# ANRGUSC/DEFER

Measured on NVIDIA H100. Metric: inferences_per_sec, higher is better.
Workload: dtype bf16x3->f32

## Files before the change

### defer_b200/csrc/conv_umma.cu

```cuda
#include <cuda.h>
#include <string.h>

#include <type_traits>

#include <vector>

#include "common.cuh"
#include "conv_umma.cuh"

namespace defer {

static int env_int(const char* name, int dflt) {
  const char* v = getenv(name);
  return v ? atoi(v) : dflt;
}

namespace {

constexpr int BM = 128;
constexpr int BK = 64;
constexpr int CONS_THREADS = 256;
constexpr int NUM_THREADS = CONS_THREADS + 128;
constexpr int SMEM_CAP = 227 * 1024 - 256;
constexpr int CTL_BYTES = 256;
// ... 214 lines not shown
struct EpiArgs {
  const float* scale;
  const float* shift;
  const __nv_bfloat16* res;
  __nv_bfloat16* y;
  size_t plane;
  int cout;
  bool relu;
  bool store_first;
  bool relu2;
  const float* scale2;
  const float* shift2;
  __nv_bfloat16* y2;
};

__device__ __forceinline__ EpiArgs epi_args(const MegaOp& op) {
  const KParams& p = op.p;
  EpiArgs e;
  e.scale = p.scale;
  e.shift = p.shift;
  e.res = reinterpret_cast<const __nv_bfloat16*>(p.res);
  e.y = reinterpret_cast<__nv_bfloat16*>(p.y);
  e.plane = p.plane_out;
  e.cout = p.cout;
  e.relu = (p.flags & DEFER_FLAG_RELU) != 0;
  e.store_first = op.store_first != 0;
  e.relu2 = op.relu2 != 0;
  e.scale2 = op.scale2;
  e.shift2 = op.shift2;
  e.y2 = reinterpret_cast<__nv_bfloat16*>(op.y2);
  return e;
}

__device__ __forceinline__ uint32_t stg_off(int r, int c) {
  return (uint32_t)(r * STG_COLS + (((c >> 2) ^ ((r & 7) << 1)) << 2) + (c & 3)) * 4u;
}
__device__ __forceinline__ void sts2(uint32_t addr, float a, float b) {
  asm volatile("st.shared.v2.f32 [%0], {%1, %2};" ::"r"(addr), "f"(a), "f"(b));
}
__device__ __forceinline__ float4 lds4(uint32_t addr) {
  float4 v;
  asm volatile("ld.shared.v4.f32 {%0, %1, %2, %3}, [%4];" : "=f"(v.x), "=f"(v.y), "=f"(v.z), "=f"(v.w) : "r"(addr));
  return v;
}
__device__ __forceinline__ void stg4(void* p, uint4 v) {
  asm volatile("st.global.v4.b32 [%0], {%1, %2, %3, %4};" ::"l"(p), "r"(v.x), "r"(v.y), "r"(v.z), "r"(v.w));
}

__device__ __forceinline__ float bf_lo(uint32_t w) { return __uint_as_float(w << 16); }
__device__ __forceinline__ float bf_hi(uint32_t w) { return __uint_as_float(w & 0xffff0000u); }

template <int NPLANES, int BN, bool AFF>
__device__ __forceinline__ void epi_tile(const KParams& p, const EpiArgs& e, uint32_t stg, const float (&acc)[BN / 2],
                                         uint32_t qmask, int c_base, int n0, int h0, int w0) {
  const int tid = threadIdx.x;
  const int lane = tid & 31;
  const int row0 = (tid >> 7) * 64 + ((tid >> 5) & 3) * 16 + (lane >> 2);
  const int col_l = 2 * (lane & 3);
  const int jg = tid & 7;
  const int rb = tid >> 3;
  const int ca = 2 * jg + ((jg >> 2) & 1), cb = ca ^ 1;
  const bool swap = (jg >> 2) & 1;
  size_t orow[4];
  uint32_t vmask = 0;
#pragma unroll
  for (int k = 0; k < 4; ++k) {
    bool v;
    size_t pix;
    row_to_pixel(p, rb + 32 * k, n0, h0, w0, v, pix);
    orow[k] = pix * (size_t)e.cout;
    vmask |= (uint32_t)v << k;
  }
#pragma unroll
  for (int P = 0; P < BN / STG_COLS; ++P) {
    const bool mine = (qmask >> (8 * P + jg)) & 1u;
    const int c = c_base + STG_COLS * P + 8 * jg;
    cons_bar_sync();
#pragma unroll
    for (int qq = 0; qq < 8; ++qq) {
      const int q = 8 * P + qq;
      if (!((qmask >> q) & 1u)) continue;
      sts2(stg + stg_off(row0, 8 * qq + col_l), acc[4 * q], acc[4 * q + 1]);
      sts2(stg + stg_off(row0 + 8, 8 * qq + col_l), acc[4 * q + 2], acc[4 * q + 3]);
    }
    uint4 rh[4], rl[4];
#pragma unroll
    for (int k = 0; k < 4; ++k) {
      rh[k] = rl[k] = make_uint4(0u, 0u, 0u, 0u);
      if (e.res && mine && ((vmask >> k) & 1u)) {
        rh[k] = __ldcg(reinterpret_cast<const uint4*>(e.res + orow[k] + c));
        if (NPLANES == 2) rl[k] = __ldcg(reinterpret_cast<const uint4*>(e.res + e.plane + orow[k] + c));
      }
    }
    float sc[8], sf[8];
#pragma unroll
    for (int i = 0; i < 8; ++i) { sc[i] = 1.f; sf[i] = 0.f; }
    if (mine) {
      if (e.scale) {
        const float4 a = __ldg(reinterpret_cast<const float4*>(e.scale + c));
        const float4 b = __ldg(reinterpret_cast<const float4*>(e.scale + c + 4));
        sc[0] = a.x; sc[1] = a.y; sc[2] = a.z; sc[3] = a.w; sc[4] = b.x; sc[5] = b.y; sc[6] = b.z; sc[7] = b.w;
      }
      if (e.shift) {
        const float4 a = __ldg(reinterpret_cast<const float4*>(e.shift + c));
        const float4 b = __ldg(reinterpret_cast<const float4*>(e.shift + c + 4));
        sf[0] = a.x; sf[1] = a.y; sf[2] = a.z; sf[3] = a.w; sf[4] = b.x; sf[5] = b.y; sf[6] = b.z; sf[7] = b.w;
      }
    }
    cons_bar_sync();
    if (!mine) continue;

#pragma unroll
    for (int k = 0; k < 4; ++k) {
      if (!((vmask >> k) & 1u)) continue;
      const int r = rb + 32 * k;
      const float4 xa = lds4(stg + stg_off(r, 4 * ca));
      const float4 xb = lds4(stg + stg_off(r, 4 * cb));
      const float4 x0 = swap ? xb : xa, x1 = swap ? xa : xb;
      float v[8] = {x0.x, x0.y, x0.z, x0.w, x1.x, x1.y, x1.z, x1.w};
      const uint32_t hw[4] = {rh[k].x, rh[k].y, rh[k].z, rh[k].w};
      const uint32_t lw[4] = {rl[k].x, rl[k].y, rl[k].z, rl[k].w};
#pragma unroll
      for (int i = 0; i < 8; ++i) {
        v[i] = fmaf(v[i], sc[i], sf[i]);
        if (e.res) {
          v[i] += (i & 1) ? bf_hi(hw[i >> 1]) : bf_lo(hw[i >> 1]);
          if (NPLANES == 2) v[i] += (i & 1) ? bf_hi(lw[i >> 1]) : bf_lo(lw[i >> 1]);
        }
        if (e.relu) v[i] = fmaxf(v[i], 0.f);
      }
      uint4 hi, lo = make_uint4(0u, 0u, 0u, 0u);
      if (NPLANES == 2) {
        split_bf16x2(v[0], v[1], hi.x, lo.x);
        split_bf16x2(v[2], v[3], hi.y, lo.y);
        split_bf16x2(v[4], v[5], hi.z, lo.z);
        split_bf16x2(v[6], v[7], hi.w, lo.w);
      } else {
        hi = make_uint4(pack_bf16x2(v[0], v[1]), pack_bf16x2(v[2], v[3]), pack_bf16x2(v[4], v[5]), pack_bf16x2(v[6], v[7]));
      }
      const size_t o = orow[k] + c;
      if (!AFF || e.store_first) {
        stg4(e.y + o, hi);
        if (NPLANES == 2) stg4(e.y + e.plane + o, lo);
      }
      if constexpr (AFF) {
        float s2[8], t2[8];
        {
          const float4 a = __ldg(reinterpret_cast<const float4*>(e.scale2 + c));
          const float4 b = __ldg(reinterpret_cast<const float4*>(e.scale2 + c + 4));
          const float4 d = __ldg(reinterpret_cast<const float4*>(e.shift2 + c));
          const float4 f = __ldg(reinterpret_cast<const float4*>(e.shift2 + c + 4));
          s2[0] = a.x; s2[1] = a.y; s2[2] = a.z; s2[3] = a.w; s2[4] = b.x; s2[5] = b.y; s2[6] = b.z; s2[7] = b.w;
          t2[0] = d.x; t2[1] = d.y; t2[2] = d.z; t2[3] = d.w; t2[4] = f.x; t2[5] = f.y; t2[6] = f.z; t2[7] = f.w;
        }
        const uint32_t sh[4] = {hi.x, hi.y, hi.z, hi.w};
        const uint32_t sl[4] = {lo.x, lo.y, lo.z, lo.w};
        float u[8];
#pragma unroll
        for (int i = 0; i < 8; ++i) {
          u[i] = (i & 1) ? bf_hi(sh[i >> 1]) : bf_lo(sh[i >> 1]);
          if (NPLANES == 2) u[i] = u[i] + ((i & 1) ? bf_hi(sl[i >> 1]) : bf_lo(sl[i >> 1]));
          u[i] = fmaf(u[i], s2[i], t2[i]);
          if (e.relu2) u[i] = fmaxf(u[i], 0.f);
        }
        uint4 h2, l2;
        if (NPLANES == 2) {
          split_bf16x2(u[0], u[1], h2.x, l2.x);
          split_bf16x2(u[2], u[3], h2.y, l2.y);
          split_bf16x2(u[4], u[5], h2.z, l2.z);
          split_bf16x2(u[6], u[7], h2.w, l2.w);
          stg4(e.y2 + o, h2);
          stg4(e.y2 + e.plane + o, l2);
        } else {
          h2 = make_uint4(pack_bf16x2(u[0], u[1]), pack_bf16x2(u[2], u[3]), pack_bf16x2(u[4], u[5]), pack_bf16x2(u[6], u[7]));
          stg4(e.y2 + o, h2);
        }
      }
    }
  }
}

template <int NPLANES, int BN, int MODE, bool AFF = false>
__device__ __forceinline__ void conv_body(const MegaOp* ops, int n_ops, int stages, int pdl) {
  using L = Smem<NPLANES, BN>;
  constexpr int R = BN / 2;
  extern __shared__ uint8_t smem_raw[];
  uint8_t* smem = reinterpret_cast<uint8_t*>((reinterpret_cast<uintptr_t>(smem_raw) + 1023) & ~(uintptr_t)1023);
  const uint32_t ring = smem_u32(smem);
  const bool red = MODE == 0 && ops[0].p.cluster;
  const uint32_t stg = ring + L::ring(stages, red);
  const uint32_t bar_base = stg + STG_BYTES;
  auto full_bar = [&](int s) { return bar_base + 8u * s; };
  auto empty_bar = [&](int s) { return bar_base + 8u * (stages + s); };
  __shared__ int s_is_last;

  const int tid = threadIdx.x;
  if (tid == 0) {
    for (int s = 0; s < stages; ++s) {
      mbar_init(full_bar(s), 1);
      mbar_init(empty_bar(s), CONS_THREADS / 32);
    }
    asm volatile("fence.mbarrier_init.release.cluster;" ::: "memory");
  }
  __syncthreads();
  if (pdl) {
    asm volatile("griddepcontrol.wait;" ::: "memory");
    asm volatile("griddepcontrol.launch_dependents;" ::: "memory");
  }

  uint32_t it = 0;
  for (int o = 0; o < n_ops; ++o) {
    const MegaOp& op = ops[o];
    const KParams& p = op.p;
    const int total = op.m_tiles * op.n_tiles;
    int t_first, t_step;
    if (MODE == 0) {
      t_first = blockIdx.y * op.m_tiles + blockIdx.x;
      t_step = total;
    } else if (MODE == 1) {
      t_first = blockIdx.x;
      t_step = gridDim.x;
    } else {
      t_first = (int)cluster_ctarank();
      t_step = (int)cluster_nctarank();
    }
    const int split = MODE == 0 ? (int)blockIdx.z : 0;
    const int kb_begin = (split * p.k_blocks) / p.splits;
    const int kb_end = ((split + 1) * p.k_blocks) / p.splits;

    for (int t = t_first; t < total; t += t_step) {
      const int m_tile = t % op.m_tiles;
      const int c_base = (t / op.m_tiles) * BN;
      int n0 = 0, h0 = 0, w0 = 0;
      if (p.flat) {
        w0 = m_tile * BM;
      } else {
        const int tw = m_tile % p.tiles_w;
        const int t2 = m_tile / p.tiles_w;
        n0 = (t2 / p.tiles_h) * p.tile_n;
        h0 = (t2 % p.tiles_h) * p.tile_h;
        w0 = tw * p.tile_w;
      }

      if (tid >= CONS_THREADS) {
        if (tid == CONS_THREADS) {
          const uint32_t a_rows = p.flat ? (uint32_t)BM : (uint32_t)(p.tile_n * p.tile_h * p.tile_w);
          uint32_t i2 = it;
          for (int kb = kb_begin; kb < kb_end; ++kb, ++i2) {
            const int stage = (int)(i2 % (uint32_t)stages);
            const uint32_t phase = (i2 / (uint32_t)stages) & 1u;
            mbar_wait(empty_bar(stage), phase ^ 1u, 1);
            const uint32_t a_dst = ring + stage * L::STAGE;
            const uint32_t b_dst = a_dst + NPLANES * L::A_PLANE;
            const int tap = kb / p.cblocks;
            const int cb = kb - tap * p.cblocks;
            const int khi = tap / p.kw;
            const int kwi = tap - khi * p.kw;
            int cw = w0, ch = 0, cn = 0;
            if (!p.flat) {
              cw = w0 * p.sw + kwi - p.pad_l;
              ch = h0 * p.sh + khi - p.pad_t;
              cn = n0;
            }
            mbar_arrive_expect_tx(full_bar(stage), NPLANES * (a_rows * 128u + (uint32_t)L::B_PLANE));
            tma_load_4d(a_dst, &op.tmx[0], full_bar(stage), cb * BK, cw, ch, cn);
            tma_load_3d(b_dst, &op.tmw[0], full_bar(stage), cb * BK, c_base, tap);
            if (NPLANES == 2) {
              tma_load_4d(a_dst + L::A_PLANE, &op.tmx[1], full_bar(stage), cb * BK, cw, ch, cn);
              tma_load_3d(b_dst + L::B_PLANE, &op.tmw[1], full_bar(stage), cb * BK, c_base, tap);
            }
          }
        }
        it += (uint32_t)(kb_end - kb_begin);
        continue;
      }

      const int wg = tid >> 7;
      const int lane = tid & 31;
      float acc[R];
#pragma unroll
      for (int i = 0; i < R; ++i) acc[i] = 0.f;
      int prev_stage = -1;
      for (int kb = kb_begin; kb < kb_end; ++kb, ++it) {
        const int stage = (int)(it % (uint32_t)stages);
        mbar_wait(full_bar(stage), (it / (uint32_t)stages) & 1u, 2);
        const uint32_t a_addr = ring + stage * L::STAGE + wg * (64 * 128);
        const uint32_t b_addr = ring + stage * L::STAGE + NPLANES * L::A_PLANE;
        wg_fence();
#pragma unroll
        for (int k = 0; k < BK / 16; ++k) {
          const uint64_t a_hi = make_sw128_desc(a_addr + k * 32);
          const uint64_t b_hi = make_sw128_desc(b_addr + k * 32);
          wgmma_bf16<BN>(acc, a_hi, b_hi);
          if (NPLANES == 2) {
            wgmma_bf16<BN>(acc, make_sw128_desc(a_addr + L::A_PLANE + k * 32), b_hi);
            wgmma_bf16<BN>(acc, a_hi, make_sw128_desc(b_addr + L::B_PLANE + k * 32));
          }
        }
        wg_commit();
        wg_wait<1>();
        acc_fence(acc);
        if (prev_stage >= 0 && lane == 0) mbar_arrive(empty_bar(prev_stage));
        prev_stage = stage;
      }
      wg_wait<0>();
      acc_fence(acc);
      if (prev_stage >= 0 && lane == 0) mbar_arrive(empty_bar(prev_stage));


      if (MODE == 0 && p.cluster) {
        cons_bar_sync();
        float4* red_buf = reinterpret_cast<float4*>(smem);
#pragma unroll
        for (int q = 0; q < R / 4; ++q)
          red_buf[q * CONS_THREADS + tid] = make_float4(acc[4 * q], acc[4 * q + 1], acc[4 * q + 2], acc[4 * q + 3]);
        break;
      }
      if (MODE == 0 && p.splits > 1) {
        const size_t tile_lin = (size_t)t;
        float4* mine = reinterpret_cast<float4*>(p.partial) + (tile_lin * p.splits + split) * (R / 4) * CONS_THREADS;
#pragma unroll
        for (int q = 0; q < R / 4; ++q)
          __stcg(mine + q * CONS_THREADS + tid, make_float4(acc[4 * q], acc[4 * q + 1], acc[4 * q + 2], acc[4 * q + 3]));
        __threadfence();
        cons_bar_sync();
        if (tid == 0) {
          const unsigned prev = atomicAdd(p.counters + tile_lin, 1u);
          const int last = prev == (unsigned)(p.splits - 1);
          if (last) p.counters[tile_lin] = 0;
          s_is_last = last;
        }
        cons_bar_sync();
        if (!s_is_last) continue;
        __threadfence();
#pragma unroll
        for (int i = 0; i < R; ++i) acc[i] = 0.f;
        for (int s = 0; s < p.splits; ++s) {
          const float4* src = reinterpret_cast<const float4*>(p.partial) + (tile_lin * p.splits + s) * (R / 4) * CONS_THREADS;
#pragma unroll
          for (int q = 0; q < R / 4; ++q) {
            const float4 v = __ldcg(src + q * CONS_THREADS + tid);
            acc[4 * q] += v.x; acc[4 * q + 1] += v.y; acc[4 * q + 2] += v.z; acc[4 * q + 3] += v.w;
          }
        }
      }
      epi_tile<NPLANES, BN, AFF>(p, epi_args(op), stg, acc, 0xffffu, c_base, n0, h0, w0);
    }

    if (MODE == 0 && p.cluster) {
      cluster_sync_all();
      if (tid < CONS_THREADS) {
        const int m_tile = blockIdx.x;
        int n0 = 0, h0 = 0, w0 = 0;
        if (p.flat) {
          w0 = m_tile * BM;
        } else {
          const int t2 = m_tile / p.tiles_w;
          n0 = (t2 / p.tiles_h) * p.tile_n;
          h0 = (t2 % p.tiles_h) * p.tile_h;
          w0 = (m_tile % p.tiles_w) * p.tile_w;
        }
        const int S = p.splits;
        const int rank = (int)cluster_ctarank();
        const uint32_t mine = ring + (uint32_t)tid * 16u;
        float acc[R];
        uint32_t qmask = 0;
#pragma unroll
        for (int q = 0; q < R / 4; ++q) {
          acc[4 * q] = acc[4 * q + 1] = acc[4 * q + 2] = acc[4 * q + 3] = 0.f;
          if (q % S != rank) continue;
          qmask |= 1u << q;
          const uint32_t addr = mine + (uint32_t)(q * CONS_THREADS) * 16u;
          float4 a = dsmem_ld4(dsmem_map(addr, 0));
          for (int s = 1; s < S; ++s) {
            const float4 v = dsmem_ld4(dsmem_map(addr, (uint32_t)s));
            a.x += v.x; a.y += v.y; a.z += v.z; a.w += v.w;
          }
          acc[4 * q] = a.x; acc[4 * q + 1] = a.y; acc[4 * q + 2] = a.z; acc[4 * q + 3] = a.w;
        }
        epi_tile<NPLANES, BN, AFF>(p, epi_args(op), stg, acc, qmask, (int)blockIdx.y * BN, n0, h0, w0);
      }
      cluster_sync_all();
    }
    if (MODE == 2 && o + 1 < n_ops) {
      asm volatile("fence.proxy.async.global;" ::: "memory");
      cluster_sync_all();
    }
  }
}

template <int NPLANES, int BN>
__global__ void __launch_bounds__(NUM_THREADS, 1) conv_umma_kernel(const __grid_constant__ MegaOp op, int stages, int pdl) {
  conv_body<NPLANES, BN, 0>(&op, 1, stages, pdl);
}

template <int NPLANES, int BN>
__global__ void __launch_bounds__(NUM_THREADS, 1) conv_stream_kernel(const MegaOp* __restrict__ ops, int stages, int pdl) {
  conv_body<NPLANES, BN, 1>(ops, 1, stages, pdl);
}

template <int NPLANES, int BN>
__global__ void __launch_bounds__(NUM_THREADS, 1) conv_umma_aff_kernel(const __grid_constant__ MegaOp op, int stages, int pdl) {
  conv_body<NPLANES, BN, 0, true>(&op, 1, stages, pdl);
}

template <int NPLANES, int BN>
__global__ void __launch_bounds__(NUM_THREADS, 1) conv_stream_aff_kernel(const MegaOp* __restrict__ ops, int stages, int pdl) {
  conv_body<NPLANES, BN, 1, true>(ops, 1, stages, pdl);
}

template <int NPLANES>
__global__ void __launch_bounds__(NUM_THREADS, 1) conv_mega_kernel(const MegaOp* __restrict__ ops, int n_ops, int stages) {
  conv_body<NPLANES, MEGA_BN, 2>(ops, n_ops, stages, 0);
}

enum StemIn { STEM_F32, STEM_U8_CAFFE, STEM_U8_TF };
constexpr int PROD_THREADS = NUM_THREADS - CONS_THREADS;
constexpr int STEM_WIN_BYTES = 24 * 1024;
constexpr int STEM_WIN_VALS = STEM_WIN_BYTES / 4;
constexpr int STEM_FILL = STEM_WIN_VALS / PROD_THREADS;
constexpr int STEM_TILE_W = 16;

template <int NPLANES>
struct StemSmem {
  static constexpr int STAGE = Smem<NPLANES, 64>::STAGE;
  __host__ __device__ static constexpr int total(int stages) {
    return stages * STAGE + STG_BYTES + 2 * STEM_WIN_BYTES + CTL_BYTES + 1024;
  }
  __host__ __device__ static constexpr int max_stages() {
    return (SMEM_CAP - STG_BYTES - 2 * STEM_WIN_BYTES - CTL_BYTES - 1024) / STAGE > MAX_STAGES
               ? MAX_STAGES
               : (SMEM_CAP - STG_BYTES - 2 * STEM_WIN_BYTES - CTL_BYTES - 1024) / STAGE;
  }
};
static_assert(StemSmem<2>::max_stages() == 3 && StemSmem<1>::max_stages() == 6, "stem ring depths with two image windows");
static_assert(STEM_FILL * PROD_THREADS == STEM_WIN_VALS, "the producer threads cover a whole window");

struct StemGeo {
  const float* x;
  const uint8_t* u8;
  float s0, s1, s2;
// ... 145 lines not shown
    int wb = 0;
    for (int t = blockIdx.x; t < total; t += gridDim.x, wb ^= 1) {
      const int t_next = t + (int)gridDim.x;
      if (t_next < total) {
        stem_tile_origin(p, t_next % op.m_tiles, n0, h0, w0);
        stem_fill_load<IN>(g, ptid, n0, h0, w0, raw);
      }
      prod_bar_sync();
      const uint32_t win = win0 + (uint32_t)wb * STEM_WIN_BYTES;
      const int c_base = (t / op.m_tiles) * 64;
      for (int kb = 0; kb < k_blocks; ++kb, ++it) {
        const int stage = (int)(it % (uint32_t)stages);
        mbar_wait(empty_bar(stage), ((it / (uint32_t)stages) & 1u) ^ 1u, 1);
        const uint32_t a_dst = ring + stage * L::STAGE;
        const uint32_t b_dst = a_dst + NPLANES * L::A_PLANE;
        if (ptid == 0) {
          mbar_expect_tx(full_bar(stage), NPLANES * (uint32_t)L::B_PLANE);
          tma_load_3d(b_dst, &op.tmw[0], full_bar(stage), kb * BK, c_base, 0);
          if (NPLANES == 2) tma_load_3d(b_dst + L::B_PLANE, &op.tmw[1], full_bar(stage), kb * BK, c_base, 0);
        }
        stem_build<NPLANES>(g, win, a_dst, ptid, row_base, kb);
        asm volatile("fence.proxy.async.shared::cta;" ::: "memory");
        prod_bar_sync();
        if (ptid == 0) mbar_arrive(full_bar(stage));
      }
      if (t_next < total) stem_fill_store<IN>(g, win0 + (uint32_t)(wb ^ 1) * STEM_WIN_BYTES, ptid, raw);
    }
    return;
  }

  const int wg = tid >> 7;
  const int lane = tid & 31;
  for (int t = blockIdx.x; t < total; t += gridDim.x) {
    float acc[32];
#pragma unroll
    for (int i = 0; i < 32; ++i) acc[i] = 0.f;
    int prev_stage = -1;
    for (int kb = 0; kb < k_blocks; ++kb, ++it) {
      const int stage = (int)(it % (uint32_t)stages);
      mbar_wait(full_bar(stage), (it / (uint32_t)stages) & 1u, 2);
      const uint32_t a_addr = ring + stage * L::STAGE + wg * (64 * 128);
      const uint32_t b_addr = ring + stage * L::STAGE + NPLANES * L::A_PLANE;
      wg_fence();
#pragma unroll
      for (int k = 0; k < BK / 16; ++k) {
        const uint64_t a_hi = make_sw128_desc(a_addr + k * 32);
        const uint64_t b_hi = make_sw128_desc(b_addr + k * 32);
        wgmma_bf16<64>(acc, a_hi, b_hi);
        if (NPLANES == 2) {
          wgmma_bf16<64>(acc, make_sw128_desc(a_addr + L::A_PLANE + k * 32), b_hi);
          wgmma_bf16<64>(acc, a_hi, make_sw128_desc(b_addr + L::B_PLANE + k * 32));
        }
      }
      wg_commit();
      wg_wait<1>();
      acc_fence(acc);
      if (prev_stage >= 0 && lane == 0) mbar_arrive(empty_bar(prev_stage));
      prev_stage = stage;
    }
    wg_wait<0>();
    acc_fence(acc);
    if (prev_stage >= 0 && lane == 0) mbar_arrive(empty_bar(prev_stage));
    int n0, h0, w0;
    stem_tile_origin(p, t % op.m_tiles, n0, h0, w0);
    epi_tile<NPLANES, 64, false>(p, epi_args(op), stg, acc, 0xffffu, (t / op.m_tiles) * 64, n0, h0, w0);
  }
}

template <int NPLANES>
__global__ void __launch_bounds__(NUM_THREADS, 1) conv_stem_kernel(const MegaOp* __restrict__ ops, int stages, int pdl) {
  stem_body<NPLANES, STEM_F32>(ops, stages, pdl);
}

template <int NPLANES>
__global__ void __launch_bounds__(NUM_THREADS, 1) conv_stem_u8_kernel(const MegaOp* __restrict__ ops, int stages, int pdl) {
  stem_body<NPLANES, STEM_U8_CAFFE>(ops, stages, pdl);
}

template <int NPLANES>
__global__ void __launch_bounds__(NUM_THREADS, 1) conv_stem_u8tf_kernel(const MegaOp* __restrict__ ops, int stages, int pdl) {
  stem_body<NPLANES, STEM_U8_TF>(ops, stages, pdl);
}

__global__ void __launch_bounds__(256) weight_transform_kernel(const float* __restrict__ w, __nv_bfloat16* __restrict__ out,
                                                               int taps, int cin, int cout, int nplanes) {
  size_t total = (size_t)taps * cin * cout;
  size_t i = (size_t)blockIdx.x * blockDim.x + threadIdx.x;
  if (i >= total) return;
  int ci = (int)(i % cin);
  size_t t2 = i / cin;
  int co = (int)(t2 % cout);
  int tap = (int)(t2 / cout);
  float v = w[((size_t)tap * cin + ci) * cout + co];
  __nv_bfloat16 hi = __float2bfloat16_rn(v);
// ... 132 lines not shown
  kernel<<<grid, NUM_THREADS, smem, st>>>(op, stages, 0);
  DEFER_CUDA(cudaGetLastError());
  return DEFER_OK;
}

template <auto kernel>
int launch_grid(const void* dev_op, int n_tiles, int stages, size_t smem, cudaStream_t st) {
  DEFER_TRY((set_smem_attr<kernel>()));
  const int sms = sm_count();
  int grid = sms < n_tiles ? sms : n_tiles;
  const int rounds = (n_tiles + grid - 1) / grid;
  grid = (n_tiles + rounds - 1) / rounds;
  static const int pdl = env_int("DEFER_PDL", 0);
  if (pdl) {
    cudaLaunchConfig_t cfg;
    memset(&cfg, 0, sizeof cfg);
    cfg.gridDim = dim3(grid, 1, 1);
    cfg.blockDim = dim3(NUM_THREADS, 1, 1);
    cfg.dynamicSmemBytes = smem;
    cfg.stream = st;
    cudaLaunchAttribute attr[1];
    attr[0].id = cudaLaunchAttributeProgrammaticStreamSerialization;
    attr[0].val.programmaticStreamSerializationAllowed = 1;
    cfg.attrs = attr;
    cfg.numAttrs = 1;
    DEFER_CUDA(cudaLaunchKernelEx(&cfg, kernel, reinterpret_cast<const MegaOp*>(dev_op), stages, 1));
    return DEFER_OK;
  }
  kernel<<<grid, NUM_THREADS, smem, st>>>(reinterpret_cast<const MegaOp*>(dev_op), stages, 0);
  DEFER_CUDA(cudaGetLastError());
  return DEFER_OK;
}

template <int NPLANES, int BN, bool AFF = false>
int launch_persist_t(const void* dev_op, int n_tiles, int stages, cudaStream_t st) {
  using L = Smem<NPLANES, BN>;
  constexpr auto kernel = AFF ? &conv_stream_aff_kernel<NPLANES, BN> : &conv_stream_kernel<NPLANES, BN>;
  if (stages > L::max_stages()) stages = L::max_stages();
  if (stages < 2) stages = 2;
  return launch_grid<kernel>(dev_op, n_tiles, stages, (size_t)L::total(stages, false), st);
}

template <int NPLANES, int IN>
int launch_stem_t(const void* dev_op, int n_tiles, int stages, cudaStream_t st) {
  using L = StemSmem<NPLANES>;
  constexpr auto kernel = IN == STEM_U8_TF      ? &conv_stem_u8tf_kernel<NPLANES>
                          : IN == STEM_U8_CAFFE ? &conv_stem_u8_kernel<NPLANES>
                                                : &conv_stem_kernel<NPLANES>;
  if (stages > L::max_stages()) stages = L::max_stages();
  if (stages < 2) stages = 2;
  return launch_grid<kernel>(dev_op, n_tiles, stages, (size_t)L::total(stages), st);
}

template <int NPLANES>
int launch_mega_t(const void* dev_ops, int n_ops, int stages, cudaStream_t st) {
  using L = Smem<NPLANES, MEGA_BN>;
  DEFER_TRY(set_smem_attr<conv_mega_kernel<NPLANES>>(true));
  if (stages < 2) stages = 2;
  if (stages > L::max_stages()) stages = L::max_stages();
  const int cluster = umma_mega_cluster_size();
  cudaLaunchConfig_t cfg;
  memset(&cfg, 0, sizeof cfg);
  cfg.gridDim = dim3(cluster, 1, 1);
  cfg.blockDim = dim3(NUM_THREADS, 1, 1);
  cfg.dynamicSmemBytes = L::total(stages, false);
  cfg.stream = st;
  cudaLaunchAttribute attr[1];
  attr[0].id = cudaLaunchAttributeClusterDimension;
  attr[0].val.clusterDim.x = cluster;
  attr[0].val.clusterDim.y = 1;
// ... 187 lines not shown
}

size_t umma_mega_op_bytes() { return sizeof(MegaOp); }

int umma_mega_fill(void* host_dst, const UmmaConvPlan& P, const UmmaConvLaneArgs& a) {
  if (!P.ready || (P.bn != MEGA_BN && !P.stream) || P.splits != 1) {
    set_error("umma_mega_fill: plan is not a persistent-kernel plan (bn %d, splits %d)", P.bn, P.splits);
    return DEFER_ERR_STATE;
  }
  MegaOp op;
  fill_op(P, a, &op);
  memcpy(host_dst, &op, sizeof op);
  return DEFER_OK;
}

int umma_mega_cluster_size() {
  static int cached = 0;
  if (cached) return cached;
  int want = env_int("DEFER_MEGA_CLUSTER", 8);
  if (want < 1) want = 1;
  if (want > 16) want = 16;
  cached = want;
  return cached;
}

int launch_conv_persistent(int nplanes, const void* dev_op, int n_tiles, bool aff, cudaStream_t st) {
  const int stages = env_int("DEFER_PERSIST_STAGES", MAX_STAGES);
  if (aff)
    return nplanes == 2 ? launch_persist_t<2, 64, true>(dev_op, n_tiles, stages, st)
                        : launch_persist_t<1, 64, true>(dev_op, n_tiles, stages, st);
  return nplanes == 2 ? launch_persist_t<2, 64>(dev_op, n_tiles, stages, st) : launch_persist_t<1, 64>(dev_op, n_tiles, stages, st);
}

int launch_conv_stream(int nplanes, int bn, const void* dev_op, int n_tiles, int k_blocks, bool aff, cudaStream_t st) {
  (void)k_blocks;
  const int stages = env_int("DEFER_STREAM_STAGES", MAX_STAGES);
  if (aff) {
    if (bn == 128) return nplanes == 2 ? launch_persist_t<2, 128, true>(dev_op, n_tiles, stages, st)
                                       : launch_persist_t<1, 128, true>(dev_op, n_tiles, stages, st);
    if (bn == 64) return nplanes == 2 ? launch_persist_t<2, 64, true>(dev_op, n_tiles, stages, st)
                                      : launch_persist_t<1, 64, true>(dev_op, n_tiles, stages, st);
  }
  if (bn == 128) return nplanes == 2 ? launch_persist_t<2, 128>(dev_op, n_tiles, stages, st) : launch_persist_t<1, 128>(dev_op, n_tiles, stages, st);
  if (bn == 64) return nplanes == 2 ? launch_persist_t<2, 64>(dev_op, n_tiles, stages, st) : launch_persist_t<1, 64>(dev_op, n_tiles, stages, st);
  set_error("conv_stream: unsupported N tile %d", bn);
  return DEFER_ERR_INVALID;
}

static void stem_tile(int ho, int wo, int kh, int kw, int sh, int sw, int cin, int* tile_h, int* tile_w, int* win_rows,
                      int* win_cols) {
  *tile_w = wo < STEM_TILE_W ? wo : STEM_TILE_W;
  *tile_h = BM / *tile_w < ho ? BM / *tile_w : ho;
  *win_rows = (*tile_h - 1) * sh + kh;
  *win_cols = ((*tile_w - 1) * sw + kw) * cin;
}

bool umma_stem_fusable(int fmt, int cin, int ho, int wo, int cout, int kh, int kw, int sh, int sw, uint32_t flags) {
  if (fmt != FMT_BF16X2 && fmt != FMT_BF16) return false;
  if (cout != 64 || (flags & DEFER_FLAG_RESIDUAL) || kh * kw * cin > 256) return false;
  int tile_h, tile_w, win_rows, win_cols;
  stem_tile(ho, wo, kh, kw, sh, sw, cin, &tile_h, &tile_w, &win_rows, &win_cols);
  return (long long)win_rows * win_cols <= STEM_WIN_VALS;
}

int umma_mega_set_stem(void* host_op, const float* x, int h, int w, int cin, int kh, int kw, int sh, int sw, int pad_t,
                       int pad_l) {
  MegaOp* op = reinterpret_cast<MegaOp*>(host_op);
  KParams& p = op->p;
  op->stem_x = x;
  op->stem_h = h; op->stem_w = w; op->stem_cin = cin;
  op->stem_kh = kh; op->stem_kw = kw; op->stem_sh = sh; op->stem_sw = sw;
  op->stem_pad_t = pad_t; op->stem_pad_l = pad_l;
  op->stem_K = kh * kw * cin;
  stem_tile(p.ho, p.wo, kh, kw, sh, sw, cin, &p.tile_h, &p.tile_w, &op->stem_win_rows, &op->stem_win_cols);
  p.flat = 0;
  p.tile_n = 1;
  p.tiles_h = (p.ho + p.tile_h - 1) / p.tile_h;
// ... 36 lines not shown
```

Baseline: 14220.

## Add ping-pong consumer warpgroup schedule and residual L2 prefetch to stream conv

Adds an optional ping-pong mode for the persistent stream conv kernel. Each consumer warpgroup computes a full 128-row tile on alternating tiles, ordered by mbarriers, so one group's epilogue overlaps the other's MMA. Register budgets are redistributed with setmaxnreg. It also adds an L2 prefetch of the residual tile before the mainloop, which runs in stream mode regardless of the ping-pong setting. Ping-pong is selected by an environment variable that defaults off, so its extra complexity and register pressure only apply when enabled.

```diff
diff --git a/defer_b200/csrc/conv_umma.cu b/defer_b200/csrc/conv_umma.cu
--- a/defer_b200/csrc/conv_umma.cu
+++ b/defer_b200/csrc/conv_umma.cu
@@ -270,8 +270,27 @@
   return e;
 }
 
+template <int NPLANES, int BN, int G>
+__device__ __forceinline__ void prefetch_res_tile(const KParams& p, int c_base, int n0, int h0, int w0) {
+  const __nv_bfloat16* res = reinterpret_cast<const __nv_bfloat16*>(p.res);
+  if (!res) return;
+  constexpr int LINES = BM * (BN / 64) * NPLANES;
+  const int gt = threadIdx.x % G;
+#pragma unroll
+  for (int i = 0; i < (LINES + G - 1) / G; ++i) {
+    const int l = gt + i * G;
+    if (l >= LINES) break;
+    const int r = l % BM, q = (l / BM) % (BN / 64), pl = l / (BM * (BN / 64));
+    bool v;
+    size_t pix;
+    row_to_pixel(p, r, n0, h0, w0, v, pix);
+    if (v) asm volatile("prefetch.global.L2 [%0];" ::"l"(res + pl * p.plane_out + pix * (size_t)p.cout + c_base + 64 * q));
+  }
+}
+
+template <int SC>
 __device__ __forceinline__ uint32_t stg_off(int r, int c) {
-  return (uint32_t)(r * STG_COLS + (((c >> 2) ^ ((r & 7) << 1)) << 2) + (c & 3)) * 4u;
+  return (uint32_t)(r * SC + (((c >> 2) ^ ((r & (SC / 8 - 1)) << 1)) << 2) + (c & 3)) * 4u;
 }
 __device__ __forceinline__ void sts2(uint32_t addr, float a, float b) {
   asm volatile("st.shared.v2.f32 [%0], {%1, %2};" ::"r"(addr), "f"(a), "f"(b));
@@ -288,17 +307,25 @@
 __device__ __forceinline__ float bf_lo(uint32_t w) { return __uint_as_float(w << 16); }
 __device__ __forceinline__ float bf_hi(uint32_t w) { return __uint_as_float(w & 0xffff0000u); }
 
-template <int NPLANES, int BN, bool AFF>
-__device__ __forceinline__ void epi_tile(const KParams& p, const EpiArgs& e, uint32_t stg, const float (&acc)[BN / 2],
-                                         uint32_t qmask, int c_base, int n0, int h0, int w0) {
+template <int NPLANES, int BN, bool AFF, int G = CONS_THREADS>
+__device__ __forceinline__ void epi_tile(const KParams& p, const EpiArgs& e, uint32_t stg,
+                                         const float (&acc)[CONS_THREADS / G][BN / 2], uint32_t qmask, int c_base, int n0,
+                                         int h0, int w0) {
+  static_assert(G == CONS_THREADS || G == 128, "an epilogue group is both consumer warpgroups or one");
+  constexpr int H = CONS_THREADS / G;
+  constexpr int SC = G / 4;
+  constexpr int JG = SC / 8;
   const int tid = threadIdx.x;
+  const int gt = tid % G;
   const int lane = tid & 31;
-  const int row0 = (tid >> 7) * 64 + ((tid >> 5) & 3) * 16 + (lane >> 2);
+  const int row0 = (gt >> 7) * 64 + ((gt >> 5) & 3) * 16 + (lane >> 2);
   const int col_l = 2 * (lane & 3);
-  const int jg = tid & 7;
-  const int rb = tid >> 3;
-  const int ca = 2 * jg + ((jg >> 2) & 1), cb = ca ^ 1;
-  const bool swap = (jg >> 2) & 1;
+  const int jg = gt % JG;
+  const int rb = gt / JG;
+  const bool swap = (gt >> 2) & 1;
+  const int ca = 2 * jg + swap, cb = ca ^ 1;
+  const uint32_t bar = G == CONS_THREADS ? 1u : 3u + (uint32_t)(tid >> 7);
+  if (G != CONS_THREADS) stg += (uint32_t)(tid >> 7) * (uint32_t)(BM * SC * 4);
   size_t orow[4];
   uint32_t vmask = 0;
 #pragma unroll
@@ -310,16 +337,19 @@
     vmask |= (uint32_t)v << k;
   }
 #pragma unroll
-  for (int P = 0; P < BN / STG_COLS; ++P) {
-    const bool mine = (qmask >> (8 * P + jg)) & 1u;
-    const int c = c_base + STG_COLS * P + 8 * jg;
-    cons_bar_sync();
-#pragma unroll
-    for (int qq = 0; qq < 8; ++qq) {
-      const int q = 8 * P + qq;
+  for (int P = 0; P < BN / SC; ++P) {
+    const bool mine = (qmask >> (JG * P + jg)) & 1u;
+    const int c = c_base + SC * P + 8 * jg;
+    asm volatile("bar.sync %0, %1;" ::"r"(bar), "n"(G) : "memory");
+#pragma unroll
+    for (int qq = 0; qq < JG; ++qq) {
+      const int q = JG * P + qq;
       if (!((qmask >> q) & 1u)) continue;
-      sts2(stg + stg_off(row0, 8 * qq + col_l), acc[4 * q], acc[4 * q + 1]);
-      sts2(stg + stg_off(row0 + 8, 8 * qq + col_l), acc[4 * q + 2], acc[4 * q + 3]);
+#pragma unroll
+      for (int h = 0; h < H; ++h) {
+        sts2(stg + stg_off<SC>(row0 + 64 * h, 8 * qq + col_l), acc[h][4 * q], acc[h][4 * q + 1]);
+        sts2(stg + stg_off<SC>(row0 + 64 * h + 8, 8 * qq + col_l), acc[h][4 * q + 2], acc[h][4 * q + 3]);
+      }
     }
     uint4 rh[4], rl[4];
 #pragma unroll
@@ -345,15 +375,15 @@
         sf[0] = a.x; sf[1] = a.y; sf[2] = a.z; sf[3] = a.w; sf[4] = b.x; sf[5] = b.y; sf[6] = b.z; sf[7] = b.w;
       }
     }
-    cons_bar_sync();
+    asm volatile("bar.sync %0, %1;" ::"r"(bar), "n"(G) : "memory");
     if (!mine) continue;
 
 #pragma unroll
     for (int k = 0; k < 4; ++k) {
       if (!((vmask >> k) & 1u)) continue;
       const int r = rb + 32 * k;
-      const float4 xa = lds4(stg + stg_off(r, 4 * ca));
-      const float4 xb = lds4(stg + stg_off(r, 4 * cb));
+      const float4 xa = lds4(stg + stg_off<SC>(r, 4 * ca));
+      const float4 xb = lds4(stg + stg_off<SC>(r, 4 * cb));
       const float4 x0 = swap ? xb : xa, x1 = swap ? xa : xb;
       float v[8] = {x0.x, x0.y, x0.z, x0.w, x1.x, x1.y, x1.z, x1.w};
       const uint32_t hw[4] = {rh[k].x, rh[k].y, rh[k].z, rh[k].w};
@@ -418,10 +448,15 @@
   }
 }
 
-template <int NPLANES, int BN, int MODE, bool AFF = false>
+enum { WALK_ALL, WALK_PRODUCER, WALK_CONSUMERS };
+
+template <int NPLANES, int BN, int MODE, bool AFF = false, bool PINGPONG = false>
 __device__ __forceinline__ void conv_body(const MegaOp* ops, int n_ops, int stages, int pdl) {
   using L = Smem<NPLANES, BN>;
   constexpr int R = BN / 2;
+  constexpr bool PP = MODE == 1 && PINGPONG;
+  constexpr int H = PP ? 2 : 1;
+  constexpr int EPI_G = PP ? 128 : CONS_THREADS;
   extern __shared__ uint8_t smem_raw[];
   uint8_t* smem = reinterpret_cast<uint8_t*>((reinterpret_cast<uintptr_t>(smem_raw) + 1023) & ~(uintptr_t)1023);
   const uint32_t ring = smem_u32(smem);
@@ -430,13 +465,18 @@
   const uint32_t bar_base = stg + STG_BYTES;
   auto full_bar = [&](int s) { return bar_base + 8u * s; };
   auto empty_bar = [&](int s) { return bar_base + 8u * (stages + s); };
+  auto ord_bar = [&](int g) { return bar_base + 8u * (2 * stages + g); };
   __shared__ int s_is_last;
 
   const int tid = threadIdx.x;
   if (tid == 0) {
     for (int s = 0; s < stages; ++s) {
       mbar_init(full_bar(s), 1);
-      mbar_init(empty_bar(s), CONS_THREADS / 32);
+      mbar_init(empty_bar(s), EPI_G / 32);
+    }
+    if (PP) {
+      mbar_init(ord_bar(0), 1);
+      mbar_init(ord_bar(1), 1);
     }
     asm volatile("fence.mbarrier_init.release.cluster;" ::: "memory");
   }
@@ -445,185 +485,215 @@
     asm volatile("griddepcontrol.wait;" ::: "memory");
     asm volatile("griddepcontrol.launch_dependents;" ::: "memory");
   }
-
-  uint32_t it = 0;
-  for (int o = 0; o < n_ops; ++o) {
-    const MegaOp& op = ops[o];
-    const KParams& p = op.p;
-    const int total = op.m_tiles * op.n_tiles;
-    int t_first, t_step;
-    if (MODE == 0) {
-      t_first = blockIdx.y * op.m_tiles + blockIdx.x;
-      t_step = total;
-    } else if (MODE == 1) {
-      t_first = blockIdx.x;
-      t_step = gridDim.x;
-    } else {
-      t_first = (int)cluster_ctarank();
-      t_step = (int)cluster_nctarank();
-    }
-    const int split = MODE == 0 ? (int)blockIdx.z : 0;
-    const int kb_begin = (split * p.k_blocks) / p.splits;
-    const int kb_end = ((split + 1) * p.k_blocks) / p.splits;
-
-    for (int t = t_first; t < total; t += t_step) {
-      const int m_tile = t % op.m_tiles;
-      const int c_base = (t / op.m_tiles) * BN;
-      int n0 = 0, h0 = 0, w0 = 0;
-      if (p.flat) {
-        w0 = m_tile * BM;
+  auto walk = [&](auto role) {
+    constexpr int ROLE = decltype(role)::value;
+    uint32_t it = 0;
+    for (int o = 0; o < n_ops; ++o) {
+      const MegaOp& op = ops[o];
+      const KParams& p = op.p;
+      const int total = op.m_tiles * op.n_tiles;
+      int t_first, t_step;
+      if (MODE == 0) {
+        t_first = blockIdx.y * op.m_tiles + blockIdx.x;
+        t_step = total;
+      } else if (MODE == 1) {
+        t_first = blockIdx.x;
+        t_step = gridDim.x;
       } else {
-        const int tw = m_tile % p.tiles_w;
-        const int t2 = m_tile / p.tiles_w;
-        n0 = (t2 / p.tiles_h) * p.tile_n;
-        h0 = (t2 % p.tiles_h) * p.tile_h;
-        w0 = tw * p.tile_w;
+        t_first = (int)cluster_ctarank();
+        t_step = (int)cluster_nctarank();
       }
-
-      if (tid >= CONS_THREADS) {
-        if (tid == CONS_THREADS) {
-          const uint32_t a_rows = p.flat ? (uint32_t)BM : (uint32_t)(p.tile_n * p.tile_h * p.tile_w);
-          uint32_t i2 = it;
-          for (int kb = kb_begin; kb < kb_end; ++kb, ++i2) {
-            const int stage = (int)(i2 % (uint32_t)stages);
-            const uint32_t phase = (i2 / (uint32_t)stages) & 1u;
-            mbar_wait(empty_bar(stage), phase ^ 1u, 1);
-            const uint32_t a_dst = ring + stage * L::STAGE;
-            const uint32_t b_dst = a_dst + NPLANES * L::A_PLANE;
-            const int tap = kb / p.cblocks;
-            const int cb = kb - tap * p.cblocks;
-            const int khi = tap / p.kw;
-            const int kwi = tap - khi * p.kw;
-            int cw = w0, ch = 0, cn = 0;
-            if (!p.flat) {
-              cw = w0 * p.sw + kwi - p.pad_l;
-              ch = h0 * p.sh + khi - p.pad_t;
-              cn = n0;
+      const int split = MODE == 0 ? (int)blockIdx.z : 0;
+      const int kb_begin = (split * p.k_blocks) / p.splits;
+      const int kb_end = ((split + 1) * p.k_blocks) / p.splits;
+
+      auto origin = [&](int t, int& c_base, int& n0, int& h0, int& w0) {
+        const int m_tile = PP ? t / op.n_tiles : t % op.m_tiles;
+        c_base = (PP ? t % op.n_tiles : t / op.m_tiles) * BN;
+        n0 = h0 = w0 = 0;
+        if (p.flat) {
+          w0 = m_tile * BM;
+        } else {
+          const int tw = m_tile % p.tiles_w;
+          const int t2 = m_tile / p.tiles_w;
+          n0 = (t2 / p.tiles_h) * p.tile_n;
+          h0 = (t2 % p.tiles_h) * p.tile_h;
+          w0 = tw * p.tile_w;
+        }
+      };
+
+      for (int t = t_first, j = 0; t < total; t += t_step, ++j) {
+        int c_base, n0, h0, w0;
+        origin(t, c_base, n0, h0, w0);
+
+        if (ROLE == WALK_PRODUCER || (ROLE == WALK_ALL && tid >= CONS_THREADS)) {
+          if (tid == CONS_THREADS) {
+            const uint32_t a_rows = p.flat ? (uint32_t)BM : (uint32_t)(p.tile_n * p.tile_h * p.tile_w);
+            uint32_t i2 = it;
+            for (int kb = kb_begin; kb < kb_end; ++kb, ++i2) {
+              const int stage = (int)(i2 % (uint32_t)stages);
+              const uint32_t phase = (i2 / (uint32_t)stages) & 1u;
+              mbar_wait(empty_bar(stage), phase ^ 1u, 1);
+              const uint32_t a_dst = ring + stage * L::STAGE;
+              const uint32_t b_dst = a_dst + NPLANES * L::A_PLANE;
+              const int tap = kb / p.cblocks;
+              const int cb = kb - tap * p.cblocks;
+              const int khi = tap / p.kw;
+              const int kwi = tap - khi * p.kw;
+              int cw = w0, ch = 0, cn = 0;
+              if (!p.flat) {
+                cw = w0 * p.sw + kwi - p.pad_l;
+                ch = h0 * p.sh + khi - p.pad_t;
+                cn = n0;
+              }
+              mbar_arrive_expect_tx(full_bar(stage), NPLANES * (a_rows * 128u + (uint32_t)L::B_PLANE));
+              tma_load_4d(a_dst, &op.tmx[0], full_bar(stage), cb * BK, cw, ch, cn);
+              tma_load_3d(b_dst, &op.tmw[0], full_bar(stage), cb * BK, c_base, tap);
+              if (NPLANES == 2) {
+                tma_load_4d(a_dst + L::A_PLANE, &op.tmx[1], full_bar(stage), cb * BK, cw, ch, cn);
+                tma_load_3d(b_dst + L::B_PLANE, &op.tmw[1], full_bar(stage), cb * BK, c_base, tap);
+              }
             }
-            mbar_arrive_expect_tx(full_bar(stage), NPLANES * (a_rows * 128u + (uint32_t)L::B_PLANE));
-            tma_load_4d(a_dst, &op.tmx[0], full_bar(stage), cb * BK, cw, ch, cn);
-            tma_load_3d(b_dst, &op.tmw[0], full_bar(stage), cb * BK, c_base, tap);
-            if (NPLANES == 2) {
-              tma_load_4d(a_dst + L::A_PLANE, &op.tmx[1], full_bar(stage), cb * BK, cw, ch, cn);
-              tma_load_3d(b_dst + L::B_PLANE, &op.tmw[1], full_bar(stage), cb * BK, c_base, tap);
+          }
+          it += (uint32_t)(kb_end - kb_begin);
+          continue;
+        }
+
+        const int wg = tid >> 7;
+        const int lane = tid & 31;
+        if (PP && (j & 1) != wg) {
+          it += (uint32_t)(kb_end - kb_begin);
+          continue;
+        }
+        if (MODE == 1) prefetch_res_tile<NPLANES, BN, EPI_G>(p, c_base, n0, h0, w0);
+        if (PP && j > 0) mbar_wait(ord_bar(wg ^ 1), (uint32_t)((j - 1) >> 1) & 1u, 3);
+        float acc[H][R];
+#pragma unroll
+        for (int h = 0; h < H; ++h)
+#pragma unroll
+          for (int i = 0; i < R; ++i) acc[h][i] = 0.f;
+        int prev_stage = -1;
+        for (int kb = kb_begin; kb < kb_end; ++kb, ++it) {
+          const int stage = (int)(it % (uint32_t)stages);
+          mbar_wait(full_bar(stage), (it / (uint32_t)stages) & 1u, 2);
+          const uint32_t a_addr = ring + stage * L::STAGE + (PP ? 0 : wg * (64 * 128));
+          const uint32_t b_addr = ring + stage * L::STAGE + NPLANES * L::A_PLANE;
+          wg_fence();
+#pragma unroll
+          for (int k = 0; k < BK / 16; ++k) {
+            const uint64_t b_hi = make_sw128_desc(b_addr + k * 32);
+#pragma unroll
+            for (int h = 0; h < H; ++h) {
+              const uint64_t a_hi = make_sw128_desc(a_addr + h * (64 * 128) + k * 32);
+              wgmma_bf16<BN>(acc[h], a_hi, b_hi);
+              if (NPLANES == 2) {
+                wgmma_bf16<BN>(acc[h], make_sw128_desc(a_addr + h * (64 * 128) + L::A_PLANE + k * 32), b_hi);
+                wgmma_bf16<BN>(acc[h], a_hi, make_sw128_desc(b_addr + L::B_PLANE + k * 32));
+              }
+            }
+          }
+          wg_commit();
+          wg_wait<1>();
+#pragma unroll
+          for (int h = 0; h < H; ++h) acc_fence(acc[h]);
+          if (prev_stage >= 0 && lane == 0) mbar_arrive(empty_bar(prev_stage));
+          prev_stage = stage;
+        }
+        if (PP && (tid & 127) == 0) mbar_arrive(ord_bar(wg));
+        wg_wait<0>();
+#pragma unroll
+        for (int h = 0; h < H; ++h) acc_fence(acc[h]);
+        if (prev_stage >= 0 && lane == 0) mbar_arrive(empty_bar(prev_stage));
+
+
+        if (MODE == 0 && p.cluster) {
+          cons_bar_sync();
+          float4* red_buf = reinterpret_cast<float4*>(smem);
+#pragma unroll
+          for (int q = 0; q < R / 4; ++q)
+            red_buf[q * CONS_THREADS + tid] = make_float4(acc[0][4 * q], acc[0][4 * q + 1], acc[0][4 * q + 2], acc[0][4 * q + 3]);
+          break;
+        }
+        if (MODE == 0 && p.splits > 1) {
+          const size_t tile_lin = (size_t)t;
+          float4* mine = reinterpret_cast<float4*>(p.partial) + (tile_lin * p.splits + split) * (R / 4) * CONS_THREADS;
+#pragma unroll
+          for (int q = 0; q < R / 4; ++q)
+            __stcg(mine + q * CONS_THREADS + tid, make_float4(acc[0][4 * q], acc[0][4 * q + 1], acc[0][4 * q + 2], acc[0][4 * q + 3]));
+          __threadfence();
+          cons_bar_sync();
+          if (tid == 0) {
+            const unsigned prev = atomicAdd(p.counters + tile_lin, 1u);
+            const int last = prev == (unsigned)(p.splits - 1);
+            if (last) p.counters[tile_lin] = 0;
+            s_is_last = last;
+          }
+          cons_bar_sync();
+          if (!s_is_last) continue;
+          __threadfence();
+#pragma unroll
+          for (int i = 0; i < R; ++i) acc[0][i] = 0.f;
+          for (int s = 0; s < p.splits; ++s) {
+            const float4* src = reinterpret_cast<const float4*>(p.partial) + (tile_lin * p.splits + s) * (R / 4) * CONS_THREADS;
+#pragma unroll
+            for (int q = 0; q < R / 4; ++q) {
+              const float4 v = __ldcg(src + q * CONS_THREADS + tid);
+              acc[0][4 * q] += v.x; acc[0][4 * q + 1] += v.y; acc[0][4 * q + 2] += v.z; acc[0][4 * q + 3] += v.w;
             }
           }
         }
-        it += (uint32_t)(kb_end - kb_begin);
-        continue;
+        epi_tile<NPLANES, BN, AFF, EPI_G>(p, epi_args(op), stg, acc, 0xffffu, c_base, n0, h0, w0);
       }
 
-      const int wg = tid >> 7;
-      const int lane = tid & 31;
-      float acc[R];
-#pragma unroll
-      for (int i = 0; i < R; ++i) acc[i] = 0.f;
-      int prev_stage = -1;
-      for (int kb = kb_begin; kb < kb_end; ++kb, ++it) {
-        const int stage = (int)(it % (uint32_t)stages);
-        mbar_wait(full_bar(stage), (it / (uint32_t)stages) & 1u, 2);
-        const uint32_t a_addr = ring + stage * L::STAGE + wg * (64 * 128);
-        const uint32_t b_addr = ring + stage * L::STAGE + NPLANES * L::A_PLANE;
-        wg_fence();
-#pragma unroll
-        for (int k = 0; k < BK / 16; ++k) {
-          const uint64_t a_hi = make_sw128_desc(a_addr + k * 32);
-          const uint64_t b_hi = make_sw128_desc(b_addr + k * 32);
-          wgmma_bf16<BN>(acc, a_hi, b_hi);
-          if (NPLANES == 2) {
-            wgmma_bf16<BN>(acc, make_sw128_desc(a_addr + L::A_PLANE + k * 32), b_hi);
-            wgmma_bf16<BN>(acc, a_hi, make_sw128_desc(b_addr + L::B_PLANE + k * 32));
+      if (MODE == 0 && p.cluster) {
+        cluster_sync_all();
+        if (tid < CONS_THREADS) {
+          const int m_tile = blockIdx.x;
+          int n0 = 0, h0 = 0, w0 = 0;
+          if (p.flat) {
+            w0 = m_tile * BM;
+          } else {
+            const int t2 = m_tile / p.tiles_w;
+            n0 = (t2 / p.tiles_h) * p.tile_n;
+            h0 = (t2 % p.tiles_h) * p.tile_h;
+            w0 = (m_tile % p.tiles_w) * p.tile_w;
           }
+          const int S = p.splits;
+          const int rank = (int)cluster_ctarank();
+          const uint32_t mine = ring + (uint32_t)tid * 16u;
+          float acc[1][R];
+          uint32_t qmask = 0;
+#pragma unroll
+          for (int q = 0; q < R / 4; ++q) {
+            acc[0][4 * q] = acc[0][4 * q + 1] = acc[0][4 * q + 2] = acc[0][4 * q + 3] = 0.f;
+            if (q % S != rank) continue;
+            qmask |= 1u << q;
+            const uint32_t addr = mine + (uint32_t)(q * CONS_THREADS) * 16u;
+            float4 a = dsmem_ld4(dsmem_map(addr, 0));
+            for (int s = 1; s < S; ++s) {
+              const float4 v = dsmem_ld4(dsmem_map(addr, (uint32_t)s));
+              a.x += v.x; a.y += v.y; a.z += v.z; a.w += v.w;
+            }
+            acc[0][4 * q] = a.x; acc[0][4 * q + 1] = a.y; acc[0][4 * q + 2] = a.z; acc[0][4 * q + 3] = a.w;
+          }
+          epi_tile<NPLANES, BN, AFF>(p, epi_args(op), stg, acc, qmask, (int)blockIdx.y * BN, n0, h0, w0);
         }
-        wg_commit();
-        wg_wait<1>();
-        acc_fence(acc);
-        if (prev_stage >= 0 && lane == 0) mbar_arrive(empty_bar(prev_stage));
-        prev_stage = stage;
+        cluster_sync_all();
       }
-      wg_wait<0>();
-      acc_fence(acc);
-      if (prev_stage >= 0 && lane == 0) mbar_arrive(empty_bar(prev_stage));
-
-
-      if (MODE == 0 && p.cluster) {
-        cons_bar_sync();
-        float4* red_buf = reinterpret_cast<float4*>(smem);
-#pragma unroll
-        for (int q = 0; q < R / 4; ++q)
-          red_buf[q * CONS_THREADS + tid] = make_float4(acc[4 * q], acc[4 * q + 1], acc[4 * q + 2], acc[4 * q + 3]);
-        break;
+      if (MODE == 2 && o + 1 < n_ops) {
+        asm volatile("fence.proxy.async.global;" ::: "memory");
+        cluster_sync_all();
       }
-      if (MODE == 0 && p.splits > 1) {
-        const size_t tile_lin = (size_t)t;
-        float4* mine = reinterpret_cast<float4*>(p.partial) + (tile_lin * p.splits + split) * (R / 4) * CONS_THREADS;
-#pragma unroll
-        for (int q = 0; q < R / 4; ++q)
-          __stcg(mine + q * CONS_THREADS + tid, make_float4(acc[4 * q], acc[4 * q + 1], acc[4 * q + 2], acc[4 * q + 3]));
-        __threadfence();
-        cons_bar_sync();
-        if (tid == 0) {
-          const unsigned prev = atomicAdd(p.counters + tile_lin, 1u);
-          const int last = prev == (unsigned)(p.splits - 1);
-          if (last) p.counters[tile_lin] = 0;
-          s_is_last = last;
-        }
-        cons_bar_sync();
-        if (!s_is_last) continue;
-        __threadfence();
-#pragma unroll
-        for (int i = 0; i < R; ++i) acc[i] = 0.f;
-        for (int s = 0; s < p.splits; ++s) {
-          const float4* src = reinterpret_cast<const float4*>(p.partial) + (tile_lin * p.splits + s) * (R / 4) * CONS_THREADS;
-#pragma unroll
-          for (int q = 0; q < R / 4; ++q) {
-            const float4 v = __ldcg(src + q * CONS_THREADS + tid);
-            acc[4 * q] += v.x; acc[4 * q + 1] += v.y; acc[4 * q + 2] += v.z; acc[4 * q + 3] += v.w;
-          }
-        }
-      }
-      epi_tile<NPLANES, BN, AFF>(p, epi_args(op), stg, acc, 0xffffu, c_base, n0, h0, w0);
-    }
-
-    if (MODE == 0 && p.cluster) {
-      cluster_sync_all();
-      if (tid < CONS_THREADS) {
-        const int m_tile = blockIdx.x;
-        int n0 = 0, h0 = 0, w0 = 0;
-        if (p.flat) {
-          w0 = m_tile * BM;
-        } else {
-          const int t2 = m_tile / p.tiles_w;
-          n0 = (t2 / p.tiles_h) * p.tile_n;
-          h0 = (t2 % p.tiles_h) * p.tile_h;
-          w0 = (m_tile % p.tiles_w) * p.tile_w;
-        }
-        const int S = p.splits;
-        const int rank = (int)cluster_ctarank();
-        const uint32_t mine = ring + (uint32_t)tid * 16u;
-        float acc[R];
-        uint32_t qmask = 0;
-#pragma unroll
-        for (int q = 0; q < R / 4; ++q) {
-          acc[4 * q] = acc[4 * q + 1] = acc[4 * q + 2] = acc[4 * q + 3] = 0.f;
-          if (q % S != rank) continue;
-          qmask |= 1u << q;
-          const uint32_t addr = mine + (uint32_t)(q * CONS_THREADS) * 16u;
-          float4 a = dsmem_ld4(dsmem_map(addr, 0));
-          for (int s = 1; s < S; ++s) {
-            const float4 v = dsmem_ld4(dsmem_map(addr, (uint32_t)s));
-            a.x += v.x; a.y += v.y; a.z += v.z; a.w += v.w;
-          }
-          acc[4 * q] = a.x; acc[4 * q + 1] = a.y; acc[4 * q + 2] = a.z; acc[4 * q + 3] = a.w;
-        }
-        epi_tile<NPLANES, BN, AFF>(p, epi_args(op), stg, acc, qmask, (int)blockIdx.y * BN, n0, h0, w0);
-      }
-      cluster_sync_all();
-    }
-    if (MODE == 2 && o + 1 < n_ops) {
-      asm volatile("fence.proxy.async.global;" ::: "memory");
-      cluster_sync_all();
-    }
+    }
+  };
+  if (!PP) {
+    walk(std::integral_constant<int, WALK_ALL>());
+  } else if (tid >= CONS_THREADS) {
+    asm volatile("setmaxnreg.dec.sync.aligned.u32 40;");
+    walk(std::integral_constant<int, WALK_PRODUCER>());
+  } else {
+    asm volatile("setmaxnreg.inc.sync.aligned.u32 232;");
+    walk(std::integral_constant<int, WALK_CONSUMERS>());
   }
 }
 
@@ -632,9 +702,9 @@
   conv_body<NPLANES, BN, 0>(&op, 1, stages, pdl);
 }
 
-template <int NPLANES, int BN>
+template <int NPLANES, int BN, bool PINGPONG>
 __global__ void __launch_bounds__(NUM_THREADS, 1) conv_stream_kernel(const MegaOp* __restrict__ ops, int stages, int pdl) {
-  conv_body<NPLANES, BN, 1>(ops, 1, stages, pdl);
+  conv_body<NPLANES, BN, 1, false, PINGPONG>(ops, 1, stages, pdl);
 }
 
 template <int NPLANES, int BN>
@@ -642,9 +712,9 @@
   conv_body<NPLANES, BN, 0, true>(&op, 1, stages, pdl);
 }
 
-template <int NPLANES, int BN>
+template <int NPLANES, int BN, bool PINGPONG>
 __global__ void __launch_bounds__(NUM_THREADS, 1) conv_stream_aff_kernel(const MegaOp* __restrict__ ops, int stages, int pdl) {
-  conv_body<NPLANES, BN, 1, true>(ops, 1, stages, pdl);
+  conv_body<NPLANES, BN, 1, true, PINGPONG>(ops, 1, stages, pdl);
 }
 
 template <int NPLANES>
@@ -856,9 +926,9 @@
   const int wg = tid >> 7;
   const int lane = tid & 31;
   for (int t = blockIdx.x; t < total; t += gridDim.x) {
-    float acc[32];
-#pragma unroll
-    for (int i = 0; i < 32; ++i) acc[i] = 0.f;
+    float acc[1][32];
+#pragma unroll
+    for (int i = 0; i < 32; ++i) acc[0][i] = 0.f;
     int prev_stage = -1;
     for (int kb = 0; kb < k_blocks; ++kb, ++it) {
       const int stage = (int)(it % (uint32_t)stages);
@@ -870,20 +940,20 @@
       for (int k = 0; k < BK / 16; ++k) {
         const uint64_t a_hi = make_sw128_desc(a_addr + k * 32);
         const uint64_t b_hi = make_sw128_desc(b_addr + k * 32);
-        wgmma_bf16<64>(acc, a_hi, b_hi);
+        wgmma_bf16<64>(acc[0], a_hi, b_hi);
         if (NPLANES == 2) {
-          wgmma_bf16<64>(acc, make_sw128_desc(a_addr + L::A_PLANE + k * 32), b_hi);
-          wgmma_bf16<64>(acc, a_hi, make_sw128_desc(b_addr + L::B_PLANE + k * 32));
+          wgmma_bf16<64>(acc[0], make_sw128_desc(a_addr + L::A_PLANE + k * 32), b_hi);
+          wgmma_bf16<64>(acc[0], a_hi, make_sw128_desc(b_addr + L::B_PLANE + k * 32));
         }
       }
       wg_commit();
       wg_wait<1>();
-      acc_fence(acc);
+      acc_fence(acc[0]);
       if (prev_stage >= 0 && lane == 0) mbar_arrive(empty_bar(prev_stage));
       prev_stage = stage;
     }
     wg_wait<0>();
-    acc_fence(acc);
+    acc_fence(acc[0]);
     if (prev_stage >= 0 && lane == 0) mbar_arrive(empty_bar(prev_stage));
     int n0, h0, w0;
     stem_tile_origin(p, t % op.m_tiles, n0, h0, w0);
@@ -1082,10 +1152,10 @@
   return DEFER_OK;
 }
 
-template <int NPLANES, int BN, bool AFF = false>
+template <int NPLANES, int BN, bool AFF = false, bool PINGPONG = false>
 int launch_persist_t(const void* dev_op, int n_tiles, int stages, cudaStream_t st) {
   using L = Smem<NPLANES, BN>;
-  constexpr auto kernel = AFF ? &conv_stream_aff_kernel<NPLANES, BN> : &conv_stream_kernel<NPLANES, BN>;
+  constexpr auto kernel = AFF ? &conv_stream_aff_kernel<NPLANES, BN, PINGPONG> : &conv_stream_kernel<NPLANES, BN, PINGPONG>;
   if (stages > L::max_stages()) stages = L::max_stages();
   if (stages < 2) stages = 2;
   return launch_grid<kernel>(dev_op, n_tiles, stages, (size_t)L::total(stages, false), st);
@@ -1339,17 +1409,26 @@
   return nplanes == 2 ? launch_persist_t<2, 64>(dev_op, n_tiles, stages, st) : launch_persist_t<1, 64>(dev_op, n_tiles, stages, st);
 }
 
+template <int NPLANES, int BN, bool AFF>
+int launch_stream_t(const void* dev_op, int n_tiles, int k_blocks, int stages, cudaStream_t st) {
+  const int mode = env_int("DEFER_PINGPONG", 0);
+  const bool pp = mode == 2 || (mode == 1 && n_tiles > sm_count() && k_blocks >= env_int("DEFER_PINGPONG_MIN_KB", 4));
+  return pp ? launch_persist_t<NPLANES, BN, AFF, true>(dev_op, n_tiles, stages, st)
+            : launch_persist_t<NPLANES, BN, AFF, false>(dev_op, n_tiles, stages, st);
+}
+
 int launch_conv_stream(int nplanes, int bn, const void* dev_op, int n_tiles, int k_blocks, bool aff, cudaStream_t st) {
-  (void)k_blocks;
   const int stages = env_int("DEFER_STREAM_STAGES", MAX_STAGES);
   if (aff) {
-    if (bn == 128) return nplanes == 2 ? launch_persist_t<2, 128, true>(dev_op, n_tiles, stages, st)
-                                       : launch_persist_t<1, 128, true>(dev_op, n_tiles, stages, st);
-    if (bn == 64) return nplanes == 2 ? launch_persist_t<2, 64, true>(dev_op, n_tiles, stages, st)
-                                      : launch_persist_t<1, 64, true>(dev_op, n_tiles, stages, st);
-  }
-  if (bn == 128) return nplanes == 2 ? launch_persist_t<2, 128>(dev_op, n_tiles, stages, st) : launch_persist_t<1, 128>(dev_op, n_tiles, stages, st);
-  if (bn == 64) return nplanes == 2 ? launch_persist_t<2, 64>(dev_op, n_tiles, stages, st) : launch_persist_t<1, 64>(dev_op, n_tiles, stages, st);
+    if (bn == 128) return nplanes == 2 ? launch_stream_t<2, 128, true>(dev_op, n_tiles, k_blocks, stages, st)
+                                       : launch_stream_t<1, 128, true>(dev_op, n_tiles, k_blocks, stages, st);
+    if (bn == 64) return nplanes == 2 ? launch_stream_t<2, 64, true>(dev_op, n_tiles, k_blocks, stages, st)
+                                      : launch_stream_t<1, 64, true>(dev_op, n_tiles, k_blocks, stages, st);
+  }
+  if (bn == 128) return nplanes == 2 ? launch_stream_t<2, 128, false>(dev_op, n_tiles, k_blocks, stages, st)
+                                     : launch_stream_t<1, 128, false>(dev_op, n_tiles, k_blocks, stages, st);
+  if (bn == 64) return nplanes == 2 ? launch_stream_t<2, 64, false>(dev_op, n_tiles, k_blocks, stages, st)
+                                    : launch_stream_t<1, 64, false>(dev_op, n_tiles, k_blocks, stages, st);
   set_error("conv_stream: unsupported N tile %d", bn);
   return DEFER_ERR_INVALID;
 }
```

Result: no change. 14310 (median of 6 runs) (+0.6%).
